# ningw42/GPU_Stereo_Matching

Hardware: AMD Instinct MI355X
Metric: disparity-maps/sec + ms/frame, 1080p d_max=128 (higher is better)
Workload: dtype u8; 1 GPU; cfg3: 1920x1080 synthetic rectified pairs, 11x11 SAD box aggregation + WTA (bit-exact with getDisp/kernalFindCorr), d_max=128; the path BASELINE.md's GPU-target table and the north star's >=100x CPU BlockMatching.cpp target are quoted on; BASELINE configs[2]'s guided-filter aggregation of the same frames: 'cfg3_guided'; width=1920, height=1080, num_disp=128, radius=5, seed=1234, parallelism=frame-parallel x1

## Files before the change

### gpu_stereo_matching_amd/csrc/bm_box_mfma.hip

```cpp
#include <atomic>
#include <type_traits>

#include "bm_common.h"

namespace sm {
namespace {

typedef _Float16 h2 __attribute__((ext_vector_type(2)));
typedef _Float16 h8 __attribute__((ext_vector_type(8)));
typedef float f4 __attribute__((ext_vector_type(4)));
typedef uint32_t u4 __attribute__((ext_vector_type(4)));

constexpr int kT = 64;
constexpr int kNW = 4;
constexpr int kThreads = 64 * kNW;
constexpr int kColB = 128;
constexpr uint32_t kInfBits = 0x7F800000u;
constexpr int kQueueLdsBytes = 16;

template <int R, int DMAX, int NP>
struct MG {
    static_assert(NP == 1 || NP == 2, "one or two disparities per pass");
    static constexpr int NOB = NP == 2 ? 3 : 4;
    static constexpr int NXB = (NP == 1 || R <= 6) ? 4 : 3;
    static constexpr int TOY = NOB == 4 ? kT - 2 * R : 16 * NOB;
    static constexpr int TOX = NXB == 4 ? kT - 2 * R : 16 * NXB;
    static constexpr int FOLD = 16 * NXB + 1;
    static constexpr int RC = kT + DMAX;
    static constexpr int RS_BYTES = RC * kColB;
    static constexpr int L_BYTES = kT * kColB;
    static constexpr int LDS_BYTES = L_BYTES + RS_BYTES;
    static constexpr int BIAS = ((2 * R + 1) * 255 + 1) / 2;
    static constexpr int KEEP = RC - TOX;
    static constexpr int NEW0 = KEEP & ~3;
    static constexpr int NEW4 = (RC - NEW0) / 4;
    static constexpr int MOVE_U = (KEEP * 8 + kThreads - 1) / kThreads;
    static_assert(TOY + 2 * R <= kT && TOX + 2 * R <= kT, "every output's window lies in the input tile");
    static_assert(8 * NEW4 + 8 * (kT / 4) <= kThreads, "a carried tile stages in one pass");
    static_assert(TOY * FOLD * 4 <= L_BYTES + TOX * kColB,
                  "the fold plane aliases the left tile and the band columns the next tile drops, none it keeps");
    static_assert(BIAS < 2048 && (2 * R + 1) * 255 - BIAS < 2048, "D1 exact in f16");
    static_assert((int64_t)(2 * R + 1) * (2 * R + 1) * 255 * 256 + 255 < (1 << 24), "keys exact in f32");
};

__device__ __forceinline__ int slot(int col, int q) { return col * kColB + ((q ^ ((col >> 1) & 7)) << 4); }

__device__ __forceinline__ void stage_pack(const uint32_t (&w)[8], uint8_t* dst, int col, int q) {
#pragma unroll
    for (int b = 0; b < 4; ++b) {
        u4 v;
#pragma unroll
        for (int m = 0; m < 4; ++m)
            v[m] = 0x64006400u | ((w[2 * m] >> (8 * b)) & 0xFFu) | (((w[2 * m + 1] >> (8 * b)) & 0xFFu) << 16);
        *reinterpret_cast<u4*>(dst + slot(col + b, q)) = v;
    }
}

template <int NC4>
__device__ __forceinline__ void stage_cols(const uint8_t* img, int ytop, int xleft, int W, int H, int pitch,
                                           uint8_t* dst, int tid) {
    for (int e = tid; e < 8 * NC4; e += kThreads) {
        const int q = e / NC4, j = e - q * NC4;
        uint32_t w[8];
#pragma unroll
        for (int i = 0; i < 8; ++i) w[i] = ld_image_u32(img, ytop + 8 * q + i, xleft + 4 * j, W, H, pitch);
        stage_pack(w, dst, 4 * j, q);
    }
}

template <int NEW0, int NEW4>
struct CarriedElem {
    bool right;
    int q, col, dx;
    __device__ __forceinline__ explicit CarriedElem(int tid) {
        constexpr int NR = 8 * NEW4, NL = 8 * (kT / 4);
        const int e = min(tid, NR + NL - 1);
        right = e < NR;
        const int el = e - NR;
        q = right ? e / NEW4 : el / (kT / 4);
        dx = 4 * (right ? e - q * NEW4 : el - q * (kT / 4));
        col = (right ? NEW0 : 0) + dx;
    }
};

__device__ __forceinline__ int per_tile(int tid) {
    asm volatile("" : "+v"(tid));
    return tid;
}

constexpr uint32_t kAbsBits = 0x7FFF7FFFu;

__device__ __forceinline__ u4 abs_diff(u4 l, u4 r, uint32_t keep) {
    u4 ad;
#pragma unroll
    for (int m = 0; m < 4; ++m) {
        const uint32_t lm = l[m], rm = r[m];
        const h2 d = __builtin_bit_cast(h2, lm) - __builtin_bit_cast(h2, rm);
        ad[m] = __builtin_bit_cast(uint32_t, d) & keep;
    }
    return ad;
}

__device__ __forceinline__ uint2 pack_f16(f4 v) {
    uint2 p;
    p.x = __builtin_bit_cast(uint32_t, __builtin_amdgcn_cvt_pkrtz(v[0], v[1]));
    p.y = __builtin_bit_cast(uint32_t, __builtin_amdgcn_cvt_pkrtz(v[2], v[3]));
    return p;
}

__device__ __forceinline__ f4 mfma(u4 a, u4 b, f4 c) {
    return __builtin_amdgcn_mfma_f32_16x16x32_f16(__builtin_bit_cast(h8, a), __builtin_bit_cast(h8, b), c, 0, 0, 0);
}

template <int R, int DMAX, int NP, bool WALK, bool QUEUE>
__device__ __forceinline__ void box_mfma_tiles(const MatchArgs& a, int tiles_x, int tiles_y, int per, int rem,
                                               uint32_t* queue) {
    using G = MG<R, DMAX, NP>;
    constexpr int NXB = G::NXB, NOB = G::NOB;
    extern __shared__ __attribute__((aligned(16 * kColB))) uint8_t smem[];
    uint8_t* lsm = smem;
    uint8_t* rsm = smem + G::L_BYTES;

    const int tid = threadIdx.x;
    const int wave = __builtin_amdgcn_readfirstlane(tid >> 6);
    const int lane = tid & 63;
    const int l16 = lane & 15;
    const int g = lane >> 4;

    static_assert(!QUEUE || WALK, "a queue workgroup walks its runs");
    constexpr bool queued = QUEUE;
    const int wg = queued ? 0 : xcd_tile(blockIdx.x, gridDim.x);
    int t_begin = wg * per, t_end = t_begin + per;
    if (WALK && rem != 0) {
        t_begin += (int)((int64_t)wg * rem / (int)gridDim.x);
        t_end += (int)((int64_t)(wg + 1) * rem / (int)gridDim.x);
    }
    if constexpr (!WALK) t_end = t_begin + 1;
    uint32_t* const qword = reinterpret_cast<uint32_t*>(smem + G::LDS_BYTES);
    auto take_run = [&] {
        const uint32_t gi = (uint32_t)__builtin_amdgcn_readfirstlane((int)*qword);
        const BoxGrab run = box_queue_grab(gi, (uint32_t)per, (uint32_t)tiles_x, gridDim.x);
        t_begin = (int)run.begin;
        t_end = (int)run.end;
    };
    if constexpr (queued) {
        if (tid == 0) *qword = atomicAdd(queue, 1u);
        __syncthreads();
        take_run();
    }
    if (t_begin >= t_end) return;
    const int tiles = tiles_x * tiles_y;
    int frame = t_begin / tiles;
    int ty = (t_begin - frame * tiles) / tiles_x;
    int tx = t_begin - frame * tiles - ty * tiles_x;
    const int W = a.W, H = a.H;
    const int d_lo = a.d_lo, d_hi = a.d_hi;

    u4 bv0, bvm, bvp;
    u4 bh, bhs;
#pragma unroll
    for (int m = 0; m < 4; ++m) {
        uint32_t w0 = 0, wm = 0, wp = 0, wh = 0, ws = 0;
#pragma unroll
        for (int e = 0; e < 2; ++e) {
            const int j = 2 * m + e;
            const int dv = 8 * g + j - l16;
            const int xin = j < 4 ? 4 * g + j : 16 + 4 * g + (j - 4);
            const int dh = xin - l16;
            const int ds = (j < 4 ? 16 + 4 * g + j : 4 * g + (j - 4)) - l16;
            w0 |= (dv >= 0 && dv <= 2 * R ? 0x3C00u : 0u) << (16 * e);
            wm |= (dv - 16 >= 0 && dv - 16 <= 2 * R ? 0x3C00u : 0u) << (16 * e);
            wp |= (dv + 16 >= 0 && dv + 16 <= 2 * R ? 0x3C00u : 0u) << (16 * e);
            wh |= (dh >= 0 && dh <= 2 * R ? 0x5C00u : 0u) << (16 * e);
            ws |= (ds >= 0 && ds <= 2 * R ? 0x5C00u : 0u) << (16 * e);
        }
        bv0[m] = w0;
        bvm[m] = wm;
        bvp[m] = wp;
        bh[m] = wh;
        bhs[m] = ws;
    }
    const float nbias = -(float)G::BIAS;
    const f4 c1 = {nbias, nbias, nbias, nbias};
    const float c2base = (float)(256 * (2 * R + 1) * G::BIAS);

    const int laddr = slot(l16, g);

    bool carried = false;
#pragma unroll 1
    for (int tile = t_begin;; ++tile) {
        const int x0 = tx * G::TOX;
        const int y0 = ty * G::TOY;
        const uint8_t* Lf = a.left + (int64_t)frame * a.frame_stride;
        const uint8_t* Rf = a.right + (int64_t)frame * a.frame_stride;

        if (!carried) {
            const int band0 = x0 - R - d_lo - DMAX;
            const int st = per_tile(tid);
            stage_cols<G::RC / 4>(Rf, y0 - R, band0, W, H, a.pitch, rsm, st);
            stage_cols<kT / 4>(Lf, y0 - R, x0 - R, W, H, a.pitch, lsm, st);
        }

        uint32_t best[NOB][NXB][4];
#pragma unroll
        for (int ob = 0; ob < NOB; ++ob)
#pragma unroll
            for (int xb = 0; xb < NXB; ++xb)
#pragma unroll
                for (int i = 0; i < 4; ++i) best[ob][xb][i] = kInfBits;

        const int d_end = min(d_hi, W - x0 + 1);
        const int nd = max(d_end - d_lo, 0);
        const int dw_lo = d_lo + (wave * nd) / kNW;
        const int dw_hi = d_lo + ((wave + 1) * nd) / kNW;
        const int d_free = W - (min(x0 + G::TOX, W) - 1);
        const int d_m = (x0 - R + kT > W) ? d_lo : max(min(x0 - R, d_free) + 1, d_lo);
        const int n_free = max(min(dw_hi, d_m) - dw_lo, 0);
        const int dw_m = dw_lo + n_free - n_free % NP;

        const bool carry_next = WALK && tile + 1 < t_end && tx + 1 < tiles_x;
        const int nxl = x0 + G::TOX - R, nxr = nxl - d_lo - DMAX + G::NEW0;
        const bool prefetch = carry_next && y0 - R >= 0 && y0 - R + kT <= H && nxr >= 0 && nxl + kT <= W;
        uint32_t pw[8];
        auto issue_prefetch = [&] {
            if (prefetch) {
                const CarriedElem<G::NEW0, G::NEW4> ce(per_tile(tid));
                const uint8_t* p = (ce.right ? Rf : Lf) + (int64_t)(y0 - R + 8 * ce.q) * a.pitch +
                                   ((ce.right ? nxr : nxl) + ce.dx);
#pragma unroll
                for (int i = 0; i < 8; ++i) __builtin_memcpy(&pw[i], p + (int64_t)i * a.pitch, 4);
            }
        };
        if constexpr (NP == 1) issue_prefetch();

        __syncthreads();

        uint32_t next_grab = 0;
        const bool draw = queued && tile + 1 == t_end && tid == 0;
        if constexpr (queued) {
            if (draw) next_grab = atomicAdd(queue, 1u);
        }

        auto run = [&](auto masked_c, const int lo, const int hi) {
            constexpr bool MASKED = decltype(masked_c)::value;
#pragma unroll 1
            for (int d = lo; d < hi; d += NP) {
                const int dd[2] = {d, min(d + 1, hi - 1)};
                int raddr[NP];
                float c2v[NP];
                f4 c2[NP];
#pragma unroll
                for (int p = 0; p < NP; ++p) {
                    raddr[p] = slot(l16 + DMAX + d_lo - dd[p], g);
                    c2v[p] = c2base + (float)dd[p];
                    c2[p] = f4{c2v[p], c2v[p], c2v[p], c2v[p]};
                }
                const int laddr_d = laddr + (int)((uint32_t)d >> 31);
                u4 t[NP][NOB];
#pragma unroll
                for (int cb = 0; cb <= NXB; ++cb) {
                    if (cb < 4) {
                        const u4 l0 = *reinterpret_cast<const u4*>(lsm + laddr_d + cb * 16 * kColB);
                        const u4 l1 = *reinterpret_cast<const u4*>(lsm + (laddr_d ^ 64) + cb * 16 * kColB);
#pragma unroll
                        for (int p = 0; p < NP; ++p) {
                            const u4 r0 = *reinterpret_cast<const u4*>(rsm + raddr[p] + cb * 16 * kColB);
                            const u4 r1 = *reinterpret_cast<const u4*>(rsm + (raddr[p] ^ 64) + cb * 16 * kColB);
                            uint32_t keep = kAbsBits;
                            if constexpr (MASKED) {
                                const int c0 = __builtin_amdgcn_readfirstlane(x0 - R + 16 * cb - dd[p]);
                                keep = (uint32_t)(l16 + c0) < (uint32_t)(W - dd[p]) ? kAbsBits : 0u;
                            }
                            const u4 ad0 = abs_diff(l0, r0, keep);
                            const u4 ad1 = abs_diff(l1, r1, keep);
                            f4 sv[4];
                            sv[0] = mfma(ad0, bv0, c1);
                            sv[1] = mfma(ad0, bvm, c1);
                            sv[1] = mfma(ad1, bvp, sv[1]);
                            sv[2] = mfma(ad1, bv0, c1);
                            if constexpr (NOB == 4) sv[3] = mfma(ad1, bvm, c1);
#pragma unroll
                            for (int ob = 0; ob < NOB; ++ob) {
                                const uint2 pk = pack_f16(sv[ob]);
                                t[p][ob][2 * (cb & 1)] = pk.x;
                                t[p][ob][2 * (cb & 1) + 1] = pk.y;
                            }
                        }
                    }
                    if constexpr (NP == 2) __builtin_amdgcn_sched_barrier(0);
                    if (cb >= 1) {
                        const int xb = cb - 1;
                        f4 c2x[NP];
#pragma unroll
                        for (int p = 0; p < NP; ++p) {
                            c2x[p] = c2[p];
                            if constexpr (MASKED) {
                                const int e = __builtin_amdgcn_readfirstlane(W - x0 - 16 * xb - dd[p]) - 4 * g;
#pragma unroll
                                for (int i = 0; i < 4; ++i)
                                    c2x[p][i] = i <= e ? c2v[p] : __builtin_bit_cast(float, kInfBits);
                            }
                        }
#pragma unroll
                        for (int ob = 0; ob < NOB; ++ob) {
                            u4 o[NP];
#pragma unroll
                            for (int p = 0; p < NP; ++p)
                                o[p] = __builtin_bit_cast(u4, mfma((cb & 1) ? bh : bhs, t[p][ob], c2x[p]));
#pragma unroll
                            for (int i = 0; i < 4; ++i) {
                                uint32_t k = o[0][i];
#pragma unroll
                                for (int p = 1; p < NP; ++p) k = min(k, o[p][i]);
                                best[ob][xb][i] = min(best[ob][xb][i], k);
                            }
                        }
                    }
                    if constexpr (NP == 2) __builtin_amdgcn_sched_barrier(0);
                }
            }
        };
        auto run_paired = [&](auto np_c, const int lo, const int mid, const int hi) {
            static_assert(decltype(np_c)::value == 2 && NOB == 3, "the paired loop");
            auto slot_end = [] { __builtin_amdgcn_sched_barrier(0); };
            auto pin = [](auto& v) { asm volatile("" : "+v"(v)); };
            auto mins = [&](int ob, int x, const u4& o0, const u4& o1) {
#pragma unroll
                for (int i = 0; i < 4; ++i) best[ob][x][i] = min(best[ob][x][i], min(o0[i], o1[i]));
            };
            const int g16 = g << 4;
            auto swz = [&](int colb) { return colb + (((colb >> 4) & 0x70) ^ g16); };
            auto lds_u4 = [](int addr) { return *(const __attribute__((address_space(3))) u4*)(uint32_t)addr; };
            const int lds0 = (int)(uint32_t)(uintptr_t)(const __attribute__((address_space(3))) uint8_t*)smem;
            auto raddr_at = [&](int colb, int d, int (&ra)[2]) {
                ra[0] = swz(colb);
                ra[1] = swz(colb - (d + 1 < hi ? kColB : 0));
            };
            int rcol = lds0 + G::L_BYTES + (l16 + DMAX + d_lo - lo) * kColB;
            int raddr[2];
            raddr_at(rcol, lo, raddr);
            f4 c2[2];
#pragma unroll
            for (int p = 0; p < 2; ++p) {
                const float c2v = c2base + (float)(lo + p);
                c2[p] = f4{c2v, c2v, c2v, c2v};
            }
            const f4 two = {2.0f, 2.0f, 2.0f, 2.0f};
            int laddr_c[2] = {lds0 + laddr, (lds0 + laddr) ^ 64};
            f4 c1p = c1;
            int wd = W - mid, c0s = x0 - R - mid;
            auto pass = [&](auto masked_c, const int d) {
                constexpr bool MASKED = decltype(masked_c)::value;
                pin(laddr_c[0]);
                pin(laddr_c[1]);
                pin(c1p);
                const int one = d + 1 < hi ? 1 : 0;
                if constexpr (MASKED) {
                    asm volatile("" : "+s"(wd));
                    asm volatile("" : "+s"(c0s));
                }
                u4 t[2][NOB];
                u4 lq[2], rq[2][2];
                auto fetch_l = [&](int cb, int c) { lq[c] = lds_u4(laddr_c[c] + cb * 16 * kColB); };
                auto fetch_r = [&](int cb, int p, int c) {
                    rq[p][c] = lds_u4((raddr[p] ^ (64 * c)) + cb * 16 * kColB);
                };
                auto fetch = [&](int cb, int c) {
                    fetch_l(cb, c);
                    fetch_r(cb, 0, c);
                    fetch_r(cb, 1, c);
                };
                uint32_t keep[2] = {kAbsBits, kAbsBits};
                f4 c2x[2];
                auto mk_keep = [&](int cb, int p) {
                    if constexpr (MASKED)
                        keep[p] = (uint32_t)(l16 + (c0s + 16 * cb - p * one)) < (uint32_t)(wd - p * one) ? kAbsBits : 0u;
                };
                auto mk_c2x = [&](int xb, int p) {
                    if constexpr (MASKED) {
                        const int e4 = 4 * (wd - x0 - 16 * xb) - g16;
#pragma unroll
                        for (int i = 0; i < 4; ++i)
                            c2x[p][i] = 4 * (i + p * one) <= e4 ? c2[p][0] : __builtin_bit_cast(float, kInfBits);
                    }
                };
                auto step_addr = [&] {
                    rcol -= d + 2 < hi ? 2 * kColB : 0;
                    raddr_at(rcol, d + 2, raddr);
                    pin(raddr[0]);
                    pin(raddr[1]);
                };
                fetch(0, 0);
                mk_keep(0, 0);
                mk_keep(0, 1);
                u4 om[2];
#pragma unroll
                for (int cb = 0; cb <= NXB; ++cb) {
                    const bool s1 = cb < 4, s2 = cb >= 1;
                    const int xb = cb - 1;
                    u4 ad[2][2];
                    f4 sv[2][NOB];
                    u4 o[2][NOB];
                    auto half = [&](int p, int c, int h) {
#pragma unroll
                        for (int m = 2 * h; m < 2 * h + 2; ++m) {
                            const uint32_t lm = lq[c][m], rm = rq[p][c][m];
                            const h2 df = __builtin_bit_cast(h2, lm) - __builtin_bit_cast(h2, rm);
                            ad[p][c][m] = __builtin_bit_cast(uint32_t, df) & keep[p];
                        }
                    };
                    auto cvt = [&](int p, int ob) {
                        const uint2 pk = pack_f16(sv[p][ob]);
                        t[p][ob][2 * (cb & 1)] = pk.x;
                        t[p][ob][2 * (cb & 1) + 1] = pk.y;
                    };
                    auto stage2 = [&](int ob, int p) {
                        o[p][ob] = __builtin_bit_cast(u4, mfma((cb & 1) ? bh : bhs, t[p][ob], MASKED ? c2x[p] : c2[p]));
                    };
                    if (s1) {
                        fetch_l(cb, 1);
                        fetch_r(cb, 0, 1);
                        half(0, 0, 0);
                        half(0, 0, 1);
                        if (cb >= 2) mins(1, xb - 1, om[0], om[1]);
                        slot_end();
                        fetch_r(cb, 1, 1);
                        sv[0][0] = mfma(ad[0][0], bv0, c1p);
                        half(1, 0, 0);
                        slot_end();
                        sv[0][1] = mfma(ad[0][0], bvm, c1p);
                        half(1, 0, 1);
                        slot_end();
                        half(0, 1, 0);
                        if (cb == NXB) step_addr();
                        slot_end();
                        sv[1][0] = mfma(ad[1][0], bv0, c1p);
                        half(0, 1, 1);
                        slot_end();
                        sv[1][1] = mfma(ad[1][0], bvm, c1p);
                        half(1, 1, 0);
                        slot_end();
                        sv[0][2] = mfma(ad[0][1], bv0, c1p);
                        half(1, 1, 1);
                        slot_end();
                        sv[0][1] = mfma(ad[0][1], bvp, sv[0][1]);
                        cvt(0, 0);
                        if (s2) mk_c2x(xb, 0);
                        slot_end();
                        sv[1][2] = mfma(ad[1][1], bv0, c1p);
                        cvt(1, 0);
                        if (s2) mk_c2x(xb, 1);
                        slot_end();
                        sv[1][1] = mfma(ad[1][1], bvp, sv[1][1]);
                        cvt(0, 2);
                        slot_end();
                        if (s2) stage2(0, 0);
                        cvt(0, 1);
                        slot_end();
                        if (s2) stage2(0, 1);
                        cvt(1, 2);
                        if (cb + 1 < 4) mk_keep(cb + 1, 0);
                        slot_end();
                        if (s2) stage2(2, 0);
                        cvt(1, 1);
                        if (cb + 1 < 4) mk_keep(cb + 1, 1);
                        slot_end();
                        if (cb + 1 < 4) fetch(cb + 1, 0);
                        if (s2) {
                            stage2(1, 0);
                            slot_end();
                            stage2(2, 1);
                            mins(0, xb, o[0][0], o[1][0]);
                            slot_end();
                            stage2(1, 1);
                            slot_end();
                            mins(2, xb, o[0][2], o[1][2]);
                            slot_end();
                            om[0] = o[0][1];
                            om[1] = o[1][1];
                        }
                    } else {
                        mk_c2x(xb, 0);
                        stage2(0, 0);
                        step_addr();
                        mk_c2x(xb, 1);
                        stage2(0, 1);
                        slot_end();
                        stage2(2, 0);
                        mins(1, xb - 1, om[0], om[1]);
                        slot_end();
                        stage2(2, 1);
                        slot_end();
                        stage2(1, 0);
                        mins(0, xb, o[0][0], o[1][0]);
                        slot_end();
                        stage2(1, 1);
                        slot_end();
                        mins(2, xb, o[0][2], o[1][2]);
                        slot_end();
                        om[0] = o[0][1];
                        om[1] = o[1][1];
                    }
                }
                mins(1, NXB - 1, om[0], om[1]);
                c2[0] += two;
                c2[1] += two;
                if constexpr (MASKED) {
                    wd -= 2;
                    c0s -= 2;
                }
                slot_end();
            };
#pragma unroll 1
            for (int d = lo; d < mid; d += 2) pass(std::false_type{}, d);
#pragma unroll 1
            for (int d = mid; d < hi; d += 2) pass(std::true_type{}, d);
        };
        if constexpr (NP == 2) {
            run_paired(std::integral_constant<int, NP>{}, dw_lo, dw_m, dw_hi);
            if (!prefetch) {
#pragma unroll
                for (int i = 0; i < 8; ++i) pw[i] = 0;
            }
            issue_prefetch();
        } else {
            run(std::false_type{}, dw_lo, dw_m);
            run(std::true_type{}, dw_m, dw_hi);
        }
        if constexpr (queued) {
            if (draw) *qword = next_grab;
        }

        __syncthreads();

        uint32_t* fold = reinterpret_cast<uint32_t*>(smem);
        if (wave == 0) {
#pragma unroll
            for (int ob = 0; ob < NOB; ++ob)
#pragma unroll
                for (int xb = 0; xb < NXB; ++xb)
#pragma unroll
                    for (int i = 0; i < 4; ++i)
                        fold[(16 * ob + l16) * G::FOLD + 16 * xb + 4 * g + i] = best[ob][xb][i];
        }
        __syncthreads();
        if (wave != 0) {
#pragma unroll
            for (int ob = 0; ob < NOB; ++ob)
#pragma unroll
                for (int xb = 0; xb < NXB; ++xb)
#pragma unroll
                    for (int i = 0; i < 4; ++i)
                        atomicMin(&fold[(16 * ob + l16) * G::FOLD + 16 * xb + 4 * g + i], best[ob][xb][i]);
        }
        __syncthreads();
        uint8_t* Df = a.disp ? a.disp + (int64_t)frame * a.out_frame_stride : nullptr;
        uint32_t* Kf = a.keys ? a.keys + (int64_t)frame * W * H : nullptr;
        if (lane < G::TOX && x0 + lane < W) {
            const int ylim = min(G::TOY, H - y0);
            uint8_t* drow = Df ? Df + (int64_t)y0 * a.out_pitch + x0 + lane : nullptr;
            uint32_t* krow = Kf ? Kf + (int64_t)y0 * W + x0 + lane : nullptr;
            for (int j = wave; j < ylim; j += kNW) {
                const uint32_t kb = fold[j * G::FOLD + lane];
                const uint32_t kf = kb >= kInfBits ? 0xFFFFFFFFu : (uint32_t)__builtin_bit_cast(float, kb);
                const uint32_t k = min(kf, a.seed_key);
                if (drow) drow[(int64_t)j * a.out_pitch] = k < a.thresh_key ? (uint8_t)(k & 0xFFu) : (uint8_t)0;
                if (krow) krow[(int64_t)j * W] = k;
            }
        }

        if (tile + 1 == t_end) {
            if constexpr (!queued) break;
            take_run();
            if (t_begin >= t_end) break;
            tile = t_begin - 1;
            frame = t_begin / tiles;
            ty = (t_begin - frame * tiles) / tiles_x;
            tx = t_begin - frame * tiles - ty * tiles_x;
            carried = false;
        } else {
            carried = carry_next;
            if (++tx == tiles_x) {
                tx = 0;
                if (++ty == tiles_y) {
                    ty = 0;
                    ++frame;
                }
            }
        }
        if (!carried) {
            __syncthreads();
            continue;
        }
        const int mt = per_tile(tid);
        u4 mv[G::MOVE_U];
#pragma unroll
        for (int i = 0; i < G::MOVE_U; ++i) {
            const int u = min(mt + i * kThreads, G::KEEP * 8 - 1);
            mv[i] = *reinterpret_cast<const u4*>(rsm + slot((u >> 3) + G::TOX, u & 7));
        }
        __syncthreads();
#pragma unroll
        for (int i = 0; i < G::MOVE_U; ++i) {
            const int u = min(mt + i * kThreads, G::KEEP * 8 - 1);
            *reinterpret_cast<u4*>(rsm + slot(u >> 3, u & 7)) = mv[i];
        }
        const CarriedElem<G::NEW0, G::NEW4> ce(mt);
        if (!prefetch) {
#pragma unroll
            for (int i = 0; i < 8; ++i)
                pw[i] = ld_image_u32(ce.right ? Rf : Lf, y0 - R + 8 * ce.q + i, (ce.right ? nxr : nxl) + ce.dx, W, H,
                               a.pitch);
        }
        stage_pack(pw, ce.right ? rsm : lsm, ce.col, ce.q);
    }
}

template <int R, int DMAX, int NP>
__global__ __launch_bounds__(kThreads, 3) void box_mfma_kernel(MatchArgs a, int tiles_x, int tiles_y, int per,
                                                                int rem) {
    box_mfma_tiles<R, DMAX, NP, true, false>(a, tiles_x, tiles_y, per, rem, nullptr);
}

template <int R, int DMAX>
__global__ __launch_bounds__(kThreads, 3) void box_mfma_queue_kernel(MatchArgs a, int tiles_x, int tiles_y, int total,
                                                                      uint32_t* queue) {
    box_mfma_tiles<R, DMAX, 2, true, true>(a, tiles_x, tiles_y, total, 0, queue);
}

template <int R, int DMAX>
__global__ __launch_bounds__(kThreads, 3) void box_mfma_tile_kernel(MatchArgs a, int tiles_x, int tiles_y) {
    box_mfma_tiles<R, DMAX, 1, false, false>(a, tiles_x, tiles_y, 1, 0, nullptr);
}

constexpr int kRangesPerSlot = 16;

template <int R, int DMAX, int NP>
hipError_t launch_rdp(const MatchArgs& a, int batch, hipStream_t s, int workgroups, uint32_t* queue,
                      int queue_workgroups) {
    using G = MG<R, DMAX, NP>;
    static_assert(NP == box_mfma_np(R, NP == 1 ? 32 : DMAX) && G::TOX == box_mfma_tox(R, NP) &&
                      G::TOY == box_mfma_toy(R, NP),
                  "bm_box_plan.h states this tile");
    const int tiles_x = (a.W + G::TOX - 1) / G::TOX;
    const int tiles_y = (a.H + G::TOY - 1) / G::TOY;
    const int64_t total = (int64_t)tiles_x * tiles_y * batch;
    if (total <= 0 || total > 0x7FFFFFFF || workgroups < 0) return hipErrorInvalidValue;
    int64_t n = workgroups;
    if constexpr (NP == 1) {
        if (n == 0 || n >= total) {
            hipLaunchKernelGGL((box_mfma_tile_kernel<R, DMAX>), dim3((unsigned)total), dim3(kThreads),
                               (size_t)G::LDS_BYTES, s, a, tiles_x, tiles_y);
            return hipGetLastError();
        }
    }
    if constexpr (NP == 2) {
        if (n == 0 && queue) {
            int slots = 0;
            hipError_t e = resident_workgroups(reinterpret_cast<const void*>(&box_mfma_queue_kernel<R, DMAX>), kThreads,
                                               (size_t)G::LDS_BYTES + kQueueLdsBytes, &slots);
            if (e != hipSuccess) return e;
            const int q = box_queue_workgroups(NP, a.d_hi - a.d_lo, total, slots, workgroups, queue_workgroups);
            if (q > 0) {
                e = hipMemsetAsync(queue, 0, sizeof(uint32_t), s);
                if (e != hipSuccess) return e;
                hipLaunchKernelGGL((box_mfma_queue_kernel<R, DMAX>), dim3((unsigned)q), dim3(kThreads),
                                   (size_t)G::LDS_BYTES + kQueueLdsBytes, s, a, tiles_x, tiles_y, (int)total, queue);
                return hipGetLastError();
            }
        }
    }
    if (n == 0) {
        int slots = 0;
        hipError_t e = resident_workgroups(reinterpret_cast<const void*>(&box_mfma_kernel<R, DMAX, NP>), kThreads,
                                           (size_t)G::LDS_BYTES, &slots);
        if (e != hipSuccess) return e;
        n = (int64_t)slots * kRangesPerSlot;
    }
    if (n > total) n = total;
    hipLaunchKernelGGL((box_mfma_kernel<R, DMAX, NP>), dim3((unsigned)n), dim3(kThreads), (size_t)G::LDS_BYTES, s, a,
                       tiles_x, tiles_y, (int)(total / n), (int)(total % n));
    return hipGetLastError();
}

template <int R, int DMAX>
hipError_t launch_rd(const MatchArgs& a, int batch, hipStream_t s, int workgroups, uint32_t* queue,
                     int queue_workgroups) {
    if constexpr (DMAX == 64 && R <= 2) {
        if (a.d_hi - a.d_lo <= 32) return launch_rdp<R, DMAX, 1>(a, batch, s, workgroups, queue, queue_workgroups);
    }
    return launch_rdp<R, DMAX, 2>(a, batch, s, workgroups, queue, queue_workgroups);
}

template <int R>
hipError_t launch_r(const MatchArgs& a, int batch, hipStream_t s, int workgroups, uint32_t* queue,
                    int queue_workgroups) {
    const int dspan = a.d_hi - a.d_lo;
    if (dspan <= 64) return launch_rd<R, 64>(a, batch, s, workgroups, queue, queue_workgroups);
    if (dspan <= 128) return launch_rd<R, 128>(a, batch, s, workgroups, queue, queue_workgroups);
    if (dspan <= 192) return launch_rd<R, 192>(a, batch, s, workgroups, queue, queue_workgroups);
    return launch_rd<R, 256>(a, batch, s, workgroups, queue, queue_workgroups);
}

}

hipError_t launch_box_match_mfma(const MatchArgs& a, int batch, hipStream_t s, int workgroups, uint32_t* queue,
                                 int queue_workgroups) {
    if (!box_mfma_scope(box_geom(a, batch), a.valid_mode)) return hipErrorInvalidValue;
    return with_radius<1, kMaxFastRadius>(a.radius, hipErrorInvalidValue, [&](auto r) {
        return launch_r<decltype(r)::value>(a, batch, s, workgroups, queue, queue_workgroups);
    });
}

}
```

Before: 28430 disparity-maps/s.

## Interleave staged rows so vertical box sum uses overlapping ad views, fewer MFMAs

Changes the LDS staging row order so each k-group's eight rows are interleaved (staged_row), which lets the paired-disparity vertical aggregation build each output block's sum from one MFMA over a sliding 4-word view of a concatenated 8-word abs-diff vector. This replaces the previous two-MFMA accumulation for the middle output block (bvm + bvp chained) with a single MFMA per block, and reorders the stage-2/min pipeline to match the new output block order. It costs an asm barrier on the ad8 vector to keep the views in registers and relies on the new row permutation being consistently applied in all staging, prefetch and carry paths.

```diff
diff --git a/gpu_stereo_matching_amd/csrc/bm_box_mfma.hip b/gpu_stereo_matching_amd/csrc/bm_box_mfma.hip
--- a/gpu_stereo_matching_amd/csrc/bm_box_mfma.hip
+++ b/gpu_stereo_matching_amd/csrc/bm_box_mfma.hip
@@ -10,6 +10,7 @@
 typedef _Float16 h8 __attribute__((ext_vector_type(8)));
 typedef float f4 __attribute__((ext_vector_type(4)));
 typedef uint32_t u4 __attribute__((ext_vector_type(4)));
+typedef uint32_t u8 __attribute__((ext_vector_type(8)));
 
 constexpr int kT = 64;
 constexpr int kNW = 4;
@@ -45,6 +46,10 @@
 
 __device__ __forceinline__ int slot(int col, int q) { return col * kColB + ((q ^ ((col >> 1) & 7)) << 4); }
 
+__device__ __forceinline__ constexpr int staged_row(int q, int i) {
+    return 32 * (q >> 2) + 4 * (q & 3) + (i < 4 ? i : 12 + i);
+}
+
 __device__ __forceinline__ void stage_pack(const uint32_t (&w)[8], uint8_t* dst, int col, int q) {
 #pragma unroll
     for (int b = 0; b < 4; ++b) {
@@ -63,7 +68,7 @@
         const int q = e / NC4, j = e - q * NC4;
         uint32_t w[8];
 #pragma unroll
-        for (int i = 0; i < 8; ++i) w[i] = ld_image_u32(img, ytop + 8 * q + i, xleft + 4 * j, W, H, pitch);
+        for (int i = 0; i < 8; ++i) w[i] = ld_image_u32(img, ytop + staged_row(q, i), xleft + 4 * j, W, H, pitch);
         stage_pack(w, dst, 4 * j, q);
     }
 }
@@ -112,6 +117,13 @@
     return __builtin_amdgcn_mfma_f32_16x16x32_f16(__builtin_bit_cast(h8, a), __builtin_bit_cast(h8, b), c, 0, 0, 0);
 }
 
+__device__ __forceinline__ u4 ad_view(u8& ad, int ob) {
+    asm volatile("" : "+v"(ad));
+    return ob == 0   ? __builtin_shufflevector(ad, ad, 0, 1, 2, 3)
+           : ob == 1 ? __builtin_shufflevector(ad, ad, 2, 3, 4, 5)
+                     : __builtin_shufflevector(ad, ad, 4, 5, 6, 7);
+}
+
 template <int R, int DMAX, int NP, bool WALK, bool QUEUE>
 __device__ __forceinline__ void box_mfma_tiles(const MatchArgs& a, int tiles_x, int tiles_y, int per, int rem,
                                                uint32_t* queue) {
@@ -156,26 +168,25 @@
     const int W = a.W, H = a.H;
     const int d_lo = a.d_lo, d_hi = a.d_hi;
 
-    u4 bv0, bvm, bvp;
+    u4 bv, bv4, bvp;
     u4 bh, bhs;
 #pragma unroll
     for (int m = 0; m < 4; ++m) {
-        uint32_t w0 = 0, wm = 0, wp = 0, wh = 0, ws = 0;
+        uint32_t wv = 0, w4 = 0, wp = 0, wh = 0, ws = 0;
 #pragma unroll
         for (int e = 0; e < 2; ++e) {
             const int j = 2 * m + e;
-            const int dv = 8 * g + j - l16;
             const int xin = j < 4 ? 4 * g + j : 16 + 4 * g + (j - 4);
             const int dh = xin - l16;
             const int ds = (j < 4 ? 16 + 4 * g + j : 4 * g + (j - 4)) - l16;
-            w0 |= (dv >= 0 && dv <= 2 * R ? 0x3C00u : 0u) << (16 * e);
-            wm |= (dv - 16 >= 0 && dv - 16 <= 2 * R ? 0x3C00u : 0u) << (16 * e);
-            wp |= (dv + 16 >= 0 && dv + 16 <= 2 * R ? 0x3C00u : 0u) << (16 * e);
+            wv |= (dh >= 0 && dh <= 2 * R ? 0x3C00u : 0u) << (16 * e);
+            w4 |= (dh - 16 >= 0 && dh - 16 <= 2 * R ? 0x3C00u : 0u) << (16 * e);
+            wp |= (dh + 16 >= 0 && dh + 16 <= 2 * R ? 0x3C00u : 0u) << (16 * e);
             wh |= (dh >= 0 && dh <= 2 * R ? 0x5C00u : 0u) << (16 * e);
             ws |= (ds >= 0 && ds <= 2 * R ? 0x5C00u : 0u) << (16 * e);
         }
-        bv0[m] = w0;
-        bvm[m] = wm;
+        bv[m] = wv;
+        bv4[m] = w4;
         bvp[m] = wp;
         bh[m] = wh;
         bhs[m] = ws;
@@ -225,10 +236,10 @@
         auto issue_prefetch = [&] {
             if (prefetch) {
                 const CarriedElem<G::NEW0, G::NEW4> ce(per_tile(tid));
-                const uint8_t* p = (ce.right ? Rf : Lf) + (int64_t)(y0 - R + 8 * ce.q) * a.pitch +
+                const uint8_t* p = (ce.right ? Rf : Lf) + (int64_t)(y0 - R + staged_row(ce.q, 0)) * a.pitch +
                                    ((ce.right ? nxr : nxl) + ce.dx);
 #pragma unroll
-                for (int i = 0; i < 8; ++i) __builtin_memcpy(&pw[i], p + (int64_t)i * a.pitch, 4);
+                for (int i = 0; i < 8; ++i) __builtin_memcpy(&pw[i], p + (int64_t)staged_row(0, i) * a.pitch, 4);
             }
         };
         if constexpr (NP == 1) issue_prefetch();
@@ -274,11 +285,11 @@
                             const u4 ad0 = abs_diff(l0, r0, keep);
                             const u4 ad1 = abs_diff(l1, r1, keep);
                             f4 sv[4];
-                            sv[0] = mfma(ad0, bv0, c1);
-                            sv[1] = mfma(ad0, bvm, c1);
+                            sv[0] = mfma(ad0, bv, c1);
+                            sv[1] = mfma(ad0, bv4, c1);
                             sv[1] = mfma(ad1, bvp, sv[1]);
-                            sv[2] = mfma(ad1, bv0, c1);
-                            if constexpr (NOB == 4) sv[3] = mfma(ad1, bvm, c1);
+                            sv[2] = mfma(ad1, bv, c1);
+                            if constexpr (NOB == 4) sv[3] = mfma(ad1, bv4, c1);
 #pragma unroll
                             for (int ob = 0; ob < NOB; ++ob) {
                                 const uint2 pk = pack_f16(sv[ob]);
@@ -348,6 +359,7 @@
             const f4 two = {2.0f, 2.0f, 2.0f, 2.0f};
             int laddr_c[2] = {lds0 + laddr, (lds0 + laddr) ^ 64};
             f4 c1p = c1;
+            u8 ad8[2] = {};
             int wd = W - mid, c0s = x0 - R - mid;
             auto pass = [&](auto masked_c, const int d) {
                 constexpr bool MASKED = decltype(masked_c)::value;
@@ -398,7 +410,6 @@
                 for (int cb = 0; cb <= NXB; ++cb) {
                     const bool s1 = cb < 4, s2 = cb >= 1;
                     const int xb = cb - 1;
-                    u4 ad[2][2];
                     f4 sv[2][NOB];
                     u4 o[2][NOB];
                     auto half = [&](int p, int c, int h) {
@@ -406,9 +417,10 @@
                         for (int m = 2 * h; m < 2 * h + 2; ++m) {
                             const uint32_t lm = lq[c][m], rm = rq[p][c][m];
                             const h2 df = __builtin_bit_cast(h2, lm) - __builtin_bit_cast(h2, rm);
-                            ad[p][c][m] = __builtin_bit_cast(uint32_t, df) & keep[p];
+                            ad8[p][4 * c + m] = __builtin_bit_cast(uint32_t, df) & keep[p];
                         }
                     };
+                    auto stage1 = [&](int p, int ob) { sv[p][ob] = mfma(ad_view(ad8[p], ob), bv, c1p); };
                     auto cvt = [&](int p, int ob) {
                         const uint2 pk = pack_f16(sv[p][ob]);
                         t[p][ob][2 * (cb & 1)] = pk.x;
@@ -422,62 +434,58 @@
                         fetch_r(cb, 0, 1);
                         half(0, 0, 0);
                         half(0, 0, 1);
-                        if (cb >= 2) mins(1, xb - 1, om[0], om[1]);
+                        if (cb >= 2) mins(2, xb - 1, om[0], om[1]);
                         slot_end();
                         fetch_r(cb, 1, 1);
-                        sv[0][0] = mfma(ad[0][0], bv0, c1p);
+                        stage1(0, 0);
                         half(1, 0, 0);
-                        slot_end();
-                        sv[0][1] = mfma(ad[0][0], bvm, c1p);
                         half(1, 0, 1);
                         slot_end();
                         half(0, 1, 0);
                         if (cb == NXB) step_addr();
                         slot_end();
-                        sv[1][0] = mfma(ad[1][0], bv0, c1p);
+                        stage1(1, 0);
+                        half(1, 1, 0);
+                        slot_end();
+                        stage1(0, 1);
                         half(0, 1, 1);
                         slot_end();
-                        sv[1][1] = mfma(ad[1][0], bvm, c1p);
-                        half(1, 1, 0);
-                        slot_end();
-                        sv[0][2] = mfma(ad[0][1], bv0, c1p);
+                        stage1(1, 1);
                         half(1, 1, 1);
                         slot_end();
-                        sv[0][1] = mfma(ad[0][1], bvp, sv[0][1]);
+                        stage1(0, 2);
                         cvt(0, 0);
                         if (s2) mk_c2x(xb, 0);
                         slot_end();
-                        sv[1][2] = mfma(ad[1][1], bv0, c1p);
+                        stage1(1, 2);
                         cvt(1, 0);
                         if (s2) mk_c2x(xb, 1);
                         slot_end();
-                        sv[1][1] = mfma(ad[1][1], bvp, sv[1][1]);
-                        cvt(0, 2);
-                        slot_end();
                         if (s2) stage2(0, 0);
                         cvt(0, 1);
                         slot_end();
                         if (s2) stage2(0, 1);
+                        cvt(1, 1);
+                        if (cb + 1 < 4) mk_keep(cb + 1, 0);
+                        slot_end();
+                        if (s2) stage2(1, 0);
+                        cvt(0, 2);
+                        if (cb + 1 < 4) mk_keep(cb + 1, 1);
+                        slot_end();
+                        if (s2) stage2(1, 1);
                         cvt(1, 2);
-                        if (cb + 1 < 4) mk_keep(cb + 1, 0);
-                        slot_end();
-                        if (s2) stage2(2, 0);
-                        cvt(1, 1);
-                        if (cb + 1 < 4) mk_keep(cb + 1, 1);
                         slot_end();
                         if (cb + 1 < 4) fetch(cb + 1, 0);
                         if (s2) {
-                            stage2(1, 0);
+                            stage2(2, 0);
+                            mins(0, xb, o[0][0], o[1][0]);
                             slot_end();
                             stage2(2, 1);
-                            mins(0, xb, o[0][0], o[1][0]);
                             slot_end();
-                            stage2(1, 1);
+                            mins(1, xb, o[0][1], o[1][1]);
                             slot_end();
-                            mins(2, xb, o[0][2], o[1][2]);
-                            slot_end();
-                            om[0] = o[0][1];
-                            om[1] = o[1][1];
+                            om[0] = o[0][2];
+                            om[1] = o[1][2];
                         }
                     } else {
                         mk_c2x(xb, 0);
@@ -486,23 +494,23 @@
                         mk_c2x(xb, 1);
                         stage2(0, 1);
                         slot_end();
+                        stage2(1, 0);
+                        mins(2, xb - 1, om[0], om[1]);
+                        slot_end();
+                        stage2(1, 1);
+                        slot_end();
                         stage2(2, 0);
-                        mins(1, xb - 1, om[0], om[1]);
+                        mins(0, xb, o[0][0], o[1][0]);
                         slot_end();
                         stage2(2, 1);
                         slot_end();
-                        stage2(1, 0);
-                        mins(0, xb, o[0][0], o[1][0]);
-                        slot_end();
-                        stage2(1, 1);
-                        slot_end();
-                        mins(2, xb, o[0][2], o[1][2]);
-                        slot_end();
-                        om[0] = o[0][1];
-                        om[1] = o[1][1];
+                        mins(1, xb, o[0][1], o[1][1]);
+                        slot_end();
+                        om[0] = o[0][2];
+                        om[1] = o[1][2];
                     }
                 }
-                mins(1, NXB - 1, om[0], om[1]);
+                mins(2, NXB - 1, om[0], om[1]);
                 c2[0] += two;
                 c2[1] += two;
                 if constexpr (MASKED) {
@@ -609,8 +617,8 @@
         if (!prefetch) {
 #pragma unroll
             for (int i = 0; i < 8; ++i)
-                pw[i] = ld_image_u32(ce.right ? Rf : Lf, y0 - R + 8 * ce.q + i, (ce.right ? nxr : nxl) + ce.dx, W, H,
-                               a.pitch);
+                pw[i] = ld_image_u32(ce.right ? Rf : Lf, y0 - R + staged_row(ce.q, i), (ce.right ? nxr : nxl) + ce.dx,
+                                     W, H, a.pitch);
         }
         stage_pack(pw, ce.right ? rsm : lsm, ce.col, ce.q);
     }
```

Result: faster. 29660 disparity-maps/s (median of 6 runs) (+4.3%).
